# jfjell/Octree-Raymarcher

Hardware: AMD Instinct MI355X
Metric: Mrays/s (primary+shadow) at 1920x1080, depth-12 SVO (higher is better)
Workload: dtype f32; 1 GPU; c3_1080p_depth12_4x1x4_shadow; depth_per_chunk=12, chunksize=128, nodes=99473656, bricks=34206642, hbm_pool_bytes=11087035656, kernel=auto, launches_in_flight=2, frames_per_launch=16, frames_in_flight=32, gather=False, partition=single, ranks_seen=1, launcher=single process

## Files before the change

octree-raymarcher_amd/csrc/device.hip:

```cpp
#include <hip/hip_runtime.h>

#include <algorithm>
#include <cmath>
#include <cstdlib>
#include <chrono>
#include <cstring>
#include <mutex>
#include <new>
#include <string>
#include <vector>

#include "kernel_literal.hip.h"
#include "kernel_stack.hip.h"
#include "see_through.hip.h"
#include "local_shadows.hip.h"
#include "shadowmap.hip.h"
#include "locate.hip.h"
#include "ao.hip.h"
#include "hit_voxels.hip.h"
#include "hip_own.h"
#include "wide_tree.hip.h"

using namespace svo;

// ... 567 lines not shown
        uint64_t tl = std::min<uint64_t>(tree_left, desc->trees), tr = std::min<uint64_t>(std::max(tree_right, tree_left), desc->trees);
        uint64_t bl = std::min<uint64_t>(twig_left, desc->twigs), br = std::min<uint64_t>(std::max(twig_right, twig_left), desc->twigs);
        if (desc->trees > old_trees) { tl = std::min(tl, old_trees); tr = desc->trees; }
        if (desc->twigs > old_twigs) { bl = std::min(bl, old_twigs); br = desc->twigs; }
        const uint64_t keep_t = std::min(tr, old_trees), keep_b = std::min(br, old_twigs);
        std::vector<uint32_t> undo_t(cur.tree.begin() + (ptrdiff_t)std::min(tl, keep_t), cur.tree.begin() + (ptrdiff_t)keep_t);
        std::vector<uint16_t> undo_b(cur.twig.begin() + (ptrdiff_t)(std::min(bl, keep_b) * TWIG_WORDS), cur.twig.begin() + (ptrdiff_t)(keep_b * TWIG_WORDS));
        cur.tree.resize(desc->trees);
        cur.twig.resize(desc->twigs * TWIG_WORDS);
        if (tl < tr) std::memcpy(cur.tree.data() + tl, desc->tree + tl, (tr - tl) * sizeof(uint32_t));
        if (bl < br) std::memcpy(cur.twig.data() + bl * TWIG_WORDS, desc->twig + bl * TWIG_WORDS, (br - bl) * TWIG_WORDS * sizeof(uint16_t));
        const uint64_t cap_t0 = cur.tree_capacity, cap_b0 = cur.twig_capacity;
        cur.fit_capacity(cur.tree.size(), cur.twig_count());
        rc = validate_chunk(cur, why);
        if (rc != SVO_OK) {
            cur.tree.resize(old_trees); cur.twig.resize(old_twigs * TWIG_WORDS);
            std::copy(undo_t.begin(), undo_t.end(), cur.tree.begin() + (ptrdiff_t)std::min(tl, keep_t));
            std::copy(undo_b.begin(), undo_b.end(), cur.twig.begin() + (ptrdiff_t)(std::min(bl, keep_b) * TWIG_WORDS));
            cur.tree_capacity = cap_t0; cur.twig_capacity = cap_b0;
            set_error("svo_world_update: " + why); return rc;
        }
        tree_left = tl; tree_right = tr; twig_left = bl; twig_right = br;
    } else {
        ChunkPools next;
        std::memcpy(next.position, desc->position, sizeof next.position);
        next.size = desc->size; next.depth = desc->depth;
        next.tree.assign(desc->tree, desc->tree + desc->trees);
        if (desc->twigs) next.twig.assign(desc->twig, desc->twig + desc->twigs * TWIG_WORDS);
        next.tree_capacity = cur.tree_capacity;
        next.twig_capacity = cur.twig_capacity;
        next.fit_capacity(next.tree.size(), next.twig_count());
        rc = validate_chunk(next, why);
        if (rc != SVO_OK) { set_error("svo_world_update: " + why); return rc; }
        if (next.size != (float)w->chunksize) { set_error("svo_world_update: chunk size must equal chunksize"); return SVO_ERR_UNSUPPORTED; }
        cur.tree.swap(next.tree);
        cur.twig.swap(next.twig);
        cur.twigs_on_device = 0;
        cur.trees_on_device = 0;
        std::memcpy(cur.position, next.position, sizeof cur.position);
        cur.size = next.size; cur.depth = next.depth;
        cur.tree_capacity = next.tree_capacity; cur.twig_capacity = next.twig_capacity;
        if (realloc_ || desc->trees != old_trees || desc->twigs != old_twigs) { tree_left = 0; tree_right = desc->trees; twig_left = 0; twig_right = desc->twigs; }
    }
    classify_world(*w);
    if (w->device < 0) return SVO_OK;
    return install_chunk(*w, chunk, cur.tree.data(), cur.twig.data(), hipMemcpyHostToDevice, tree_left, tree_right, twig_left, twig_right);
}

}

extern "C" {

int svo_world_upload(svo_world *w, int device)
{
    try { return world_upload_impl(w, device); }
    catch (const std::bad_alloc &) { set_error("svo_world_upload: out of host memory"); return SVO_ERR_OUT_OF_MEMORY; }
    catch (...) { set_error("svo_world_upload: unexpected exception"); return SVO_ERR_HIP; }
}

int svo_world_update(svo_world *w, int chunk, const svo_chunk_desc *desc,
                     uint64_t tree_left, uint64_t tree_right, uint64_t twig_left, uint64_t twig_right, int realloc_)
{
    try { return world_update_impl(w, chunk, desc, tree_left, tree_right, twig_left, twig_right, realloc_); }
    catch (const std::bad_alloc &) { set_error("svo_world_update: out of host memory"); return SVO_ERR_OUT_OF_MEMORY; }
    catch (...) { set_error("svo_world_update: unexpected exception"); return SVO_ERR_HIP; }
}

}

namespace svo {

constexpr int STACK_REFILL = 8;
constexpr int STACK_WAVES = 6;
using StackKernel = void (*)(TraceArgs);
template <int MAXLV, bool BIG, bool GLSL, bool SEG> constexpr StackKernel stack_kernel = k_trace_stack<MAXLV, STACK_REFILL, STACK_WAVES, BIG, GLSL, SEG>;
constexpr int STACK_CLASSES = 12;
#define STACK_PAIR(MAXLV, BIG, SEG) stack_kernel<MAXLV, BIG, true, SEG>, stack_kernel<MAXLV, BIG, false, SEG>
#define STACK_SET(SEG) STACK_PAIR(10, true, SEG), STACK_PAIR(22, true, SEG), STACK_PAIR(6, false, SEG), STACK_PAIR(10, false, SEG), STACK_PAIR(16, false, SEG), STACK_PAIR(22, false, SEG)
static const StackKernel STACK_KERNELS[] = { STACK_SET(false), STACK_SET(true) };
#undef STACK_SET
#undef STACK_PAIR
static_assert(sizeof(STACK_KERNELS) / sizeof(StackKernel) == 2 * STACK_CLASSES, "an unbounded and a bounded instantiation per class");
static_assert(sizeof(STACK_KERNELS) / sizeof(StackKernel) == sizeof(Hbm::stack_blocks) / sizeof(int), "one grid size per instantiation");

}

extern "C" {

static float world_min(const svo_world *w, int a) { return (float)(w->chunkcoordmin[a] * (int)(float)w->chunksize); }
static V3 miss_ray_origin(const svo_world *w)
{
    const float cs = (float)w->chunksize;
    return V3{ world_min(w, 0), world_min(w, 1) - (float)w->height * cs - cs, world_min(w, 2) - (float)w->depth * cs - cs };
}

static int fill_common(svo_world *w, const svo_trace_params *prm, TraceArgs &A)
{
    if (!w) return SVO_ERR_INVALID_ARG;
    if (prm && prm->see_through > 0xFFFFu) { set_error("svo_trace: see_through is a 16-bit material"); return SVO_ERR_INVALID_ARG; }
    if (w->device < 0) { set_error("svo_trace: world is not uploaded"); return SVO_ERR_NOT_UPLOADED; }
    std::memset(&A, 0, sizeof A);
    const float cs = (float)w->chunksize;
    const int dims[3] = { w->width, w->height, w->depth };
    for (int a = 0; a < 3; ++a) {
        A.worldmin[a] = world_min(w, a);
        A.worldmax[a] = (float)(w->chunkcoordmin[a] + dims[a]) * cs;
    }
    A.chunksize = cs;
    A.inv_chunksize = 1.0f / cs;
    A.dimw = w->width; A.dimh = w->height; A.dimd = w->depth;
    for (int a = 0; a < 3; ++a) {
        A.ccm[a] = w->chunkcoordmin[a];
        A.cbase[a] = positive_mod(w->chunkcoordmin[a], dims[a]);
    }
    A.chunks = w->hbm->chunks.p; A.tree = w->hbm->tree.p; A.twig = w->hbm->twig.p; A.mask = w->hbm->mask.p;
    A.wchunks = w->hbm->wchunks.p; A.wide = w->hbm->wide.p; A.wbase = w->hbm->wbase.p; A.bmat = w->hbm->bmat.p;
    if (prm && prm->semantics != SVO_SEMANTICS_CPU && prm->semantics != SVO_SEMANTICS_GLSL) { set_error("svo_trace: unknown semantics"); return SVO_ERR_INVALID_ARG; }
    const bool glsl = prm && prm->semantics == SVO_SEMANTICS_GLSL;
    A.glsl = glsl ? 1 : 0;
    A.eps = (prm && prm->eps != 0.0f) ? prm->eps : (glsl ? 1.0f / 4096.0f : 1.0f / 8192.0f);
    A.cap_chunk = (prm && prm->max_chunk_steps > 0) ? prm->max_chunk_steps : (glsl ? 256 : 1000);
    A.cap_tree = (prm && prm->max_tree_steps > 0) ? prm->max_tree_steps : (glsl ? 512 : 1000);
    A.cap_twig = (prm && prm->max_twig_steps > 0) ? prm->max_twig_steps : (glsl ? 64 : 1000);
    A.guard_eps = glsl ? A.eps : -INFINITY;
    A.leaf_back = glsl ? 0.0f : A.eps;
    A.shadow = (prm && prm->shadow) ? 1 : 0;
    A.normal_mode = (prm && prm->normal_mode == SVO_NORMAL_FACE) ? SVO_NORMAL_FACE : SVO_NORMAL_CUBE;
    float l[3] = { 1.0f, -1.0f, 0.0f };
    if (prm && (prm->light_dir[0] != 0.0f || prm->light_dir[1] != 0.0f || prm->light_dir[2] != 0.0f))
        std::memcpy(l, prm->light_dir, sizeof l);
    const float nx = -l[0], ny = -l[1], nz = -l[2];
    const float inv = 1.0f / std::sqrt(nx * nx + ny * ny + nz * nz);
    A.sdir[0] = nx * inv; A.sdir[1] = ny * inv; A.sdir[2] = nz * inv;
    A.counters = prm ? prm->counters_dev : nullptr;
    A.exact_geometry = w->exact_geometry ? 1 : 0;
    A.tile_cost = prm ? prm->tile_cost_dev : nullptr;
    A.tile_order = prm ? prm->tile_order_dev : nullptr;
    A.work = w->hbm->work.p;
    return SVO_OK;
}

static bool stack_needs_big(const svo_world *w)
{
#ifdef SVO_FORCE_WIDE64
    return true;
#else
    return w->wide_pool_cap * 64 >= (1ull << 30) || w->twig_pool_cap >= (1ull << 29);
#endif
}

static int pick_kernel(const svo_world *w, const svo_trace_params *prm, const TraceArgs &A)
{
    const int want = prm ? prm->kernel : SVO_KERNEL_AUTO;
    const bool stack_ok = w->exact_geometry && w->max_levels <= (int)WIDE_MAX_LEVELS && w->wide_ok && w->twig_pool_cap < (1ull << 32);
    if (want == SVO_KERNEL_LITERAL) return SVO_KERNEL_LITERAL;
    if (want == SVO_KERNEL_STACK) {
        if (!stack_ok) { set_error("svo_trace: SVO_KERNEL_STACK needs exact geometry, chunk depth <= 24 and the world's wide trees (svo_world_info.wide_nodes)"); return SVO_ERR_UNSUPPORTED; }
        return SVO_KERNEL_STACK;
    }
    if (want != SVO_KERNEL_AUTO) { set_error("svo_trace: unknown kernel id"); return SVO_ERR_INVALID_ARG; }
    return (stack_ok && !A.counters) ? SVO_KERNEL_STACK : SVO_KERNEL_LITERAL;
}

static int launch_stack(svo_world *w, const TraceArgs &A, int tiles_per_wave, int in_flight, hipStream_t s)
{
    const int lv = w->max_levels;
    const int depth = stack_needs_big(w) ? (lv <= 10 ? 0 : 1) : lv <= 6 ? 2 : lv <= 10 ? 3 : lv <= 16 ? 4 : 5;
    const int which = 2 * depth + (A.glsl ? 0 : 1) + (A.tmax ? STACK_CLASSES : 0);
    const StackKernel kernel = STACK_KERNELS[which];
    int &resident = w->hbm->stack_blocks[which];
    if (resident <= 0) {
        hipDeviceProp_t prop;
        if (hipGetDeviceProperties(&prop, w->device) != hipSuccess) return SVO_ERR_HIP;
        int per_cu = 0;
        if (hipOccupancyMaxActiveBlocksPerMultiprocessor(&per_cu, kernel, 64, 0) != hipSuccess || per_cu <= 0) per_cu = 16;
        resident = prop.multiProcessorCount * per_cu;
#ifdef SVO_TEST_HOOKS
        if (const char *cap = std::getenv("SVO_GRID_WAVES_PER_CU")) { const int c = std::atoi(cap); if (c > 0) resident = prop.multiProcessorCount * std::min(c, per_cu); }
#endif
    }
    const int64_t per_wave = tiles_per_wave > 1 ? tiles_per_wave : 1;
    const int64_t tiles = (int64_t)A.ntiles * (A.nframes > 0 ? A.nframes : 1);
    const int64_t slots = in_flight >= 2 ? std::max<int64_t>(1, (int64_t)resident * 2 / in_flight) : resident;
    const int blocks = (int)std::min<int64_t>((tiles + per_wave - 1) / per_wave, slots);
    hipLaunchKernelGGL(kernel, dim3((unsigned)blocks), dim3(64), 0, s, A);
    return SVO_OK;
}

static int use_view(svo_world *w, uint32_t m, TraceArgs &A, hipStream_t s)
{
    Hbm &d = *w->hbm;
    if (d.view_material != m) {
        const uint64_t n4 = w->wide_pool_len * 16, bricks = w->twig_pool_len;
        if (!d.view_wide.p) {
            if (d.view_wide.alloc(std::max<uint64_t>(n4, 1) * 4, w->device) != hipSuccess ||
                d.view_mask.alloc(std::max<uint64_t>(bricks, 1), w->device) != hipSuccess) {
                d.view_wide = Pooled<uint32_t>();
                set_error("svo_trace: hipMalloc of the see-through view failed"); return SVO_ERR_OUT_OF_MEMORY;
            }
        } else {
            for (Event &e : d.work_done) if (e.e) if (const int rc = e.wait(s)) return rc;
        }
        d.view_material = 0;
        if ((n4 + 255) / 256 > 0x7FFFFFFFull || (bricks * 8 + 255) / 256 > 0x7FFFFFFFull) { set_error("svo_trace: pools too large for one view launch"); return SVO_ERR_UNSUPPORTED; }
        if (n4) hipLaunchKernelGGL(k_view_wide, dim3((unsigned)((n4 + 255) / 256)), dim3(256), 0, s, reinterpret_cast<const uint4 *>(d.wide.p),
                                   reinterpret_cast<uint4 *>(d.view_wide.p), n4, m);
        if (bricks) hipLaunchKernelGGL(k_view_mask, dim3((unsigned)((bricks * 8 + 255) / 256)), dim3(256), 0, s, d.twig.p, d.mask.p, d.view_mask.p, bricks, m);
        HIP_TRY(hipGetLastError());
        if (const int rc = d.view_built.record(s)) return rc;
        d.view_material = m;
    } else {
        if (const int rc = d.view_built.wait(s)) return rc;
    }
    A.wide = d.view_wide.p;
    A.mask = d.view_mask.p;
    return SVO_OK;
}

static int launch(svo_world *w, const svo_trace_params *prm, TraceArgs &A, hipStream_t s)
{
    const int kernel = pick_kernel(w, prm, A);
    if (kernel < 0) return kernel;
    HIP_TRY(hipSetDevice(w->device));
    const uint32_t see = prm ? prm->see_through : 0u;
    if (see && kernel == SVO_KERNEL_STACK) {
        const int rc = use_view(w, see, A, s);
        if (rc != SVO_OK) return rc;
    }
    Hbm &d = *w->hbm;
    d.work_last = d.work_next;
    d.work_next = (d.work_next + 1) % WORK_SLOTS;
    A.work = d.work.p + WORK_SLOT_WORDS * d.work_last;
    Event &ev = d.work_done[d.work_last];
    if (const int rc = ev.wait(s)) return rc;
    HIP_TRY(hipMemsetAsync(A.work, 0, WORK_SLOT_WORDS * sizeof(unsigned long long), s));
    if (A.n <= 0) return ev.record(s) == SVO_OK ? SVO_OK : SVO_ERR_HIP;
    if (kernel == SVO_KERNEL_LITERAL) {
        const int64_t blocks = (A.n + 255) / 256;
        if (blocks > 0x7FFFFFFF) { set_error("svo_trace: too many rays for one launch"); return SVO_ERR_UNSUPPORTED; }
        const auto literal = see ? (A.tmax ? k_trace_literal<true, true> : k_trace_literal<true, false>) : (A.tmax ? k_trace_literal<false, true> : k_trace_literal<false, false>);
        hipLaunchKernelGGL(literal, dim3((unsigned)blocks), dim3(256), 0, s, A, see);
    } else {
        if (A.ntiles > (1 << 25)) { set_error("svo_trace: more than 2^31 rays in one stack-kernel launch"); return SVO_ERR_UNSUPPORTED; }
        if (A.tile_cost) HIP_TRY(hipMemsetAsync(A.tile_cost, 0, (size_t)A.ntiles * (size_t)(A.from_camera ? A.nframes : 1) * 2 * sizeof(uint32_t), s));
        const int rc = launch_stack(w, A, prm ? prm->tiles_per_wave : 0, prm ? prm->launches_in_flight : 0, s);
        if (rc != SVO_OK) { set_error("svo_trace: device query failed"); return rc; }
    }
    HIP_TRY(hipGetLastError());
    return ev.record(s);
}

static int fill_cameras(const svo_camera *cams, int nframes, TraceArgs &A)
{
    if (!cams || nframes < 1 || nframes > MAX_FRAMES) { set_error("svo_trace: between 1 and 16 cameras per launch"); return SVO_ERR_INVALID_ARG; }
    for (int f = 0; f < nframes; ++f) {
        const svo_camera &c = cams[f];
        if (c.width <= 0 || c.height <= 0) { set_error("svo_trace: bad camera"); return SVO_ERR_INVALID_ARG; }
        if (c.width != cams[0].width || c.height != cams[0].height) { set_error("svo_trace_frames: the cameras of one launch share one image size"); return SVO_ERR_INVALID_ARG; }
        A.cams[f] = frame_cam(c);
    }
    A.from_camera = 1;
    A.nframes = nframes;
    A.imgw = cams[0].width; A.imgh = cams[0].height;
    return SVO_OK;
}

static int launch_frames(svo_world *w, const svo_trace_params *prm, TraceArgs &A, const char *who, hipStream_t s)
{
    A.n = (int64_t)A.w * A.h;
    A.tiles_per_row = (A.w + TILE_W - 1) / TILE_W;
    const int64_t tiles = (int64_t)A.tiles_per_row * ((A.h + TILE_H - 1) / TILE_H);
    if (tiles * A.nframes > 0x3FFFFFFF || A.n * A.nframes > 0x7FFFFFFF) { set_error(std::string(who) + ": image too large"); return SVO_ERR_UNSUPPORTED; }
    A.ntiles = (int32_t)tiles;
    if (A.nframes == 1) return launch(w, prm, A, s);
    const int kernel = pick_kernel(w, prm, A);
    if (kernel < 0) return kernel;
    if (kernel == SVO_KERNEL_STACK) return launch(w, prm, A, s);
    if (prm && prm->counters_dev) { set_error(std::string(who) + ": work counters are per launch of one frame"); return SVO_ERR_UNSUPPORTED; }
    const int nframes = A.nframes;
    char *out = static_cast<char *>(A.out);
    for (int f = 0; f < nframes; ++f) {
        TraceArgs F = A;
        F.nframes = 1; F.cams[0] = A.cams[f];
        F.out = out + (size_t)f * (size_t)A.n * sizeof(svo_hit);
        const int rc = launch(w, prm, F, s);
        if (rc != SVO_OK) return rc;
    }
    return SVO_OK;
}

int svo_trace_frames(svo_world *w, const svo_camera *cams, int nframes, const svo_trace_params *prm,
                     int x0, int y0, int rw, int rh, svo_hit *out_dev, void *stream)
{
    TraceArgs A;
    int rc = fill_common(w, prm, A);
    if (rc != SVO_OK) return rc;
    if ((rc = fill_cameras(cams, nframes, A)) != SVO_OK) return rc;
    if (!out_dev || rw < 0 || rh < 0 || x0 < 0 || y0 < 0) { set_error("svo_trace: bad rectangle or output"); return SVO_ERR_INVALID_ARG; }
    A.x0 = x0; A.y0 = y0; A.w = rw; A.h = rh;
    A.bh = rh > 0 ? rh : 1; A.ystep = 0;
    A.out = out_dev;
    return launch_frames(w, prm, A, "svo_trace", (hipStream_t)stream);
}

int svo_trace(svo_world *w, const svo_camera *cam, const svo_trace_params *prm,
              int x0, int y0, int rw, int rh, svo_hit *out_dev, void *stream)
{
    return svo_trace_frames(w, cam, 1, prm, x0, y0, rw, rh, out_dev, stream);
}

// ... 354 lines not shown
```

octree-raymarcher_amd/csrc/kernel_stack.hip.h:

```cpp
#pragma once
#include "march.hip.h"
#include "step_asm.hip.h"

namespace svo {

constexpr int CW_ESCAPE_PENDING = (int)0x80000000;
enum : int { M_DONE = 0, M_WORLD = 1, M_HIT = 2, M_TREE = 3, M_TWIG = 4 };

constexpr int VOTE_WORLD = 8;
constexpr int VOTE_HIT = 16;
constexpr int VOTE_BUSY = 24;
constexpr int CREEP_SERIOUS = 6;
constexpr int CREEP_LANES = 8;
#define SVO_LIKELY(x) __builtin_expect(!!(x), 1)
#define SVO_UNLIKELY(x) __builtin_expect(!!(x), 0)
constexpr int STEP_EXTRA = 4;
constexpr int STEP_LANES = 8;
constexpr int DRAIN_STEPS = 8;
#ifndef SVO_SURE_MISS_WHEN
#define SVO_SURE_MISS_WHEN __builtin_amdgcn_readfirstlane(more ? 0 : 1)
#endif

__device__ __forceinline__ float recip_pow2(float x) { return __uint_as_float(0x7F000000u - __float_as_uint(x)); }

__device__ __forceinline__ int chunk_index_pow2(const TraceArgs &A, V3 p)
{
    float qx = p.x * A.inv_chunksize, qy = p.y * A.inv_chunksize, qz = p.z * A.inv_chunksize;
    if (qx < 0.0f) qx -= 1.0f;
    if (qy < 0.0f) qy -= 1.0f;
    if (qz < 0.0f) qz -= 1.0f;
    const int ix = (int)qx, iy = (int)qy, iz = (int)qz;
    const int rx = ix - A.ccm[0], ry = iy - A.ccm[1], rz = iz - A.ccm[2];
    int mx = A.cbase[0] + rx, my = A.cbase[1] + ry, mz = A.cbase[2] + rz;
    mx -= (mx >= A.dimw) ? A.dimw : 0; mx += (mx < 0) ? A.dimw : 0;
    my -= (my >= A.dimh) ? A.dimh : 0; my += (my < 0) ? A.dimh : 0;
    mz -= (mz >= A.dimd) ? A.dimd : 0; mz += (mz < 0) ? A.dimd : 0;
    return my * A.dimw * A.dimd + mz * A.dimw + mx;
}

__device__ __forceinline__ V3 cube_normal_pow2(V3 s, V3 lo, float size, float eps)
{
    const V3 hi = lo + size;
    const V3 c = (lo + hi) * 0.5f;
    const V3 p = s - c;
    const float d = fabsf(lo.x - hi.x) * 0.5f;
    const float invd = recip_pow2(d);
    const float b = 1.0f + eps;
    const float ix = (float)(int)((p.x * invd) * b), iy = (float)(int)((p.y * invd) * b), iz = (float)(int)((p.z * invd) * b);
    const float dot = ix * ix + iy * iy + iz * iz;
    float inv;
    if (dot == 1.0f) inv = 1.0f;
    else if (dot == 2.0f) inv = __uint_as_float(0x3F3504F3u);
    else if (dot == 3.0f) inv = __uint_as_float(0x3F13CD3Au);
    else inv = 1.0f / sqrtf(dot);
    return mk(ix * inv, iy * inv, iz * inv);
}

__device__ __forceinline__ uint32_t child_slot(int ux, int uy, int uz, int sh)
{
    const uint32_t bx = __builtin_amdgcn_ubfe((uint32_t)ux, (uint32_t)sh, 1u);
    const uint32_t by = __builtin_amdgcn_ubfe((uint32_t)uy, (uint32_t)sh, 1u);
    const uint32_t bz = __builtin_amdgcn_ubfe((uint32_t)uz, (uint32_t)sh, 1u);
    return ((bz << 1) + by) * 2u + bx;
}
__device__ __forceinline__ uint32_t ld_node(const uint32_t *pool, uint32_t boff)
{
    return *reinterpret_cast<const uint32_t *>(reinterpret_cast<const char *>(pool) + (size_t)boff);
}
constexpr uint32_t WIDE_PAYLOAD = (1u << 25) - 1u;
__device__ __forceinline__ uint32_t wide_slot(int ux, int uy, int uz, int sh)
{
    const uint32_t bx = __builtin_amdgcn_ubfe((uint32_t)ux, (uint32_t)sh, 2u);
    const uint32_t by = __builtin_amdgcn_ubfe((uint32_t)uy, (uint32_t)sh, 2u);
    const uint32_t bz = __builtin_amdgcn_ubfe((uint32_t)uz, (uint32_t)sh, 2u);
    return (bz << 4) | (by << 2) | bx;
}
__device__ __forceinline__ bool is_branch(uint32_t word) { return (int32_t)word < (int32_t)0xC0000000; }

__device__ __forceinline__ TraceArgs args_reloaded()
{
    auto p = __builtin_amdgcn_kernarg_segment_ptr();
    asm volatile("" : "+s"(p));
    TraceArgs T;
    __builtin_memcpy(&T, p, sizeof T);
    return T;
}
__device__ __forceinline__ FrameCam camera_reloaded(int f)
{
    auto p = __builtin_amdgcn_kernarg_segment_ptr();
    asm volatile("" : "+s"(p));
    FrameCam c;
    __builtin_memcpy(&c, (decltype(p))((const char __attribute__((address_space(4))) *)p + __builtin_offsetof(TraceArgs, cams) + (size_t)f * sizeof(FrameCam)), sizeof c);
    return c;
}

__device__ __noinline__ float brick_layer_first_touch(int k, V3 a, V3 b, V3 g, V3 bmin, float r, unsigned long long mask)
{
    const float ak = k == 0 ? a.x : k == 1 ? a.y : a.z, bk = k == 0 ? b.x : k == 1 ? b.y : b.z, mk_ = k == 0 ? bmin.x : k == 1 ? bmin.y : bmin.z;
    const float au = k == 0 ? a.y : k == 1 ? a.z : a.x, av = k == 0 ? a.z : k == 1 ? a.x : a.y;
    const float gu = k == 0 ? g.y : k == 1 ? g.z : g.x, gv = k == 0 ? g.z : k == 1 ? g.x : g.y;
    const float mu = k == 0 ? bmin.y : k == 1 ? bmin.z : bmin.x, mv = k == 0 ? bmin.z : k == 1 ? bmin.x : bmin.y;
    const int su = k == 0 ? 4 : k == 1 ? 16 : 1, sv = k == 0 ? 16 : k == 1 ? 1 : 4;
    const float delta = r * 0.0625f;
    bool ok = (ak == mk_) & (bk < 0.0f);
    ok &= (mu >= 4.0f * r) & (mv >= 4.0f * r) & (delta >= (fabsf(mu) + fabsf(mv) + 8.0f * r) * 0x1p-21f);
    ok = ok && fabsf(gu) < 1.0e30f && fabsf(gv) < 1.0e30f;
    if (!ok) return -1.0f;
    const float u0 = au - mu, v0 = av - mv;
    float first = __uint_as_float(0x7F800000u);
    bool clean = true;
    for (int cv = 0; cv < 4; ++cv) {
        const float va = ((float)cv * r - delta - v0) * gv, vb = ((float)(cv + 1) * r + delta - v0) * gv;
        const float v_in = fminf(va, vb), v_out = fmaxf(va, vb);
        for (int cu = 0; cu < 4; ++cu) {
            const bool occupied = (mask >> (cu * su + cv * sv)) & 1ull;
            const float ua = ((float)cu * r - delta - u0) * gu, ub = ((float)(cu + 1) * r + delta - u0) * gu;
            const float s_in = fmaxf(fmaxf(fminf(ua, ub), v_in), 0.0f), s_out = fminf(fmaxf(ua, ub), v_out);
            clean &= (s_in == s_in) & (s_out == s_out);
            first = (occupied & (s_in <= s_out)) ? fminf(first, s_in) : first;
        }
    }
    return clean ? first * (1.0f - 0x1p-18f) : -1.0f;
}

__device__ __forceinline__ void note_tile_cost(int outk, uint32_t steps)
{
    const TraceArgs T = args_reloaded();
    if (!T.tile_cost) return;
    const int k = outk & 0x7FFFFFFF;
    int tile, frame = 0;
    if (T.from_camera) {
        const int per = T.w * T.h;
        frame = k / per;
        const int r = k - frame * per;
        const int ly = r / T.w, lx = r - ly * T.w;
        tile = (ly / TILE_H) * T.tiles_per_row + lx / TILE_W;
    } else tile = k >> 6;
    atomicMax(&T.tile_cost[((size_t)frame * (size_t)T.ntiles + (size_t)tile) * 2 + (outk < 0 ? 1 : 0)], steps);
}

template <bool GLSL>
__device__ __forceinline__ bool past_far_end(int mode, float t, float tt_saved, float tw, float eps, float far)
{
    const float tt = mode == M_TWIG ? tt_saved : t;
    return (mode == M_TREE || mode == M_TWIG) && tw + (GLSL ? tt : tt - eps) >= far;
}

template <int MAXLV, int REFILL, int WAVES_PER_SIMD, bool BIG, bool GLSL, bool SEG = false>
__global__ __launch_bounds__(64, WAVES_PER_SIMD) void k_trace_stack(TraceArgs A)
{
    __shared__ uint32_t stk[MAXLV / 2 + 1][64];
    __shared__ float tile_ray[SEG ? 12 : 11][64];
    constexpr int CHUNK_TAB = (BIG && MAXLV <= 10) ? 128 : 64;
    __shared__ uint32_t chunk_tab[6][CHUNK_TAB];
    stk[0][threadIdx.x] = 0u;
    const int lane = threadIdx.x;
    const bool want_cost = A.tile_cost != nullptr;
    const int n_chunks = A.dimw * A.dimh * A.dimd;
    const bool chunks_in_lds = n_chunks <= CHUNK_TAB;
    if (chunks_in_lds)
        for (int i = lane; i < n_chunks; i += 64) {
            const DevWide ch = A.wchunks[i];
            chunk_tab[0][i] = __float_as_uint(ch.bmin[0]); chunk_tab[1][i] = __float_as_uint(ch.bmin[1]); chunk_tab[2][i] = __float_as_uint(ch.bmin[2]);
            chunk_tab[3][i] = ch.levels; chunk_tab[4][i] = ch.wide_off; chunk_tab[5][i] = (uint32_t)ch.twig_off;
        }
    __syncthreads();
#ifdef SVO_STACK_TIMING
    const unsigned long long t_begin = __builtin_amdgcn_s_memrealtime();
    unsigned n_iters = 0, n_tree_lanes = 0, n_twig_lanes = 0, n_world_lanes = 0;
    unsigned n_world_runs = 0, n_hit_runs = 0, n_refill = 0, n_tilegen = 0, n_fix = 0;
    unsigned n_lane_twig = 0;
    unsigned n_lane_busy = 0;
    unsigned n_creep_runs = 0, n_creep_rounds = 0, n_dbg = 0;
    unsigned n_wsteps = 0, n_lsteps = 0, n_hit_wait = 0, n_dead_wait = 0, n_wsteps_b = 0, n_lsteps_b = 0, n_world_wait = 0, n_twig_b = 0;
#endif
    [[maybe_unused]] StepStats step_stats;

    const V3 wlo = ld3(A.worldmin), whi = ld3(A.worldmax);
    const V3 sdir = ld3(A.sdir);
    const V3 sg = recip(sdir);
    const float eps = A.eps;
    const bool eps_pow2 = (__float_as_uint(eps) & 0x807FFFFFu) == 0u && __float_as_uint(eps) >= 0x00800000u && __float_as_uint(eps) < 0x7F800000u;
    const float csize = A.chunksize;

    const int tr_cols = A.tiles_per_row;
    const int tr_rows = A.ntiles / (tr_cols > 0 ? tr_cols : 1);
    const bool by_cols = tr_cols >= TILE_REGIONS;
    const int reg_q = (by_cols ? tr_cols : tr_rows) / TILE_REGIONS, reg_rem = (by_cols ? tr_cols : tr_rows) % TILE_REGIONS;
    int region = (int)(__builtin_amdgcn_s_getreg(20 | (0 << 6) | (3 << 11)) & (TILE_REGIONS - 1));
    int regions_left = TILE_REGIONS;
    int tile_first = 0;
    int tile_next = 64;
    bool more = true;
    unsigned rays_marched = 0;

    int mode = M_DONE;
    int outk = 0;
    V3 alpha = mk(0, 0, 0), beta = mk(0, 0, 1), g = mk(0, 0, 0);
    float tw = 0.0f;
    [[maybe_unused]] float far = __uint_as_float(0x7F800000u);
    int cw = 0;
    uint32_t guard = 0;
    V3 O = mk(0, 0, 0), Blo = mk(0, 0, 0);
    float res = 1.0f, t = 0.0f;
    int cnt = 0;
    float tt_saved = 0.0f, t_miss = 0.0f;
    int it_saved = 0;
    V3 clo = mk(0, 0, 0);
    WideRef<BIG> wide_b = 0;
    auto ld_wide = [&](uint32_t e) -> uint32_t {
        if constexpr (BIG) return *reinterpret_cast<const uint32_t *>((size_t)wide_b + ((size_t)e << 2));
        else return ld_node(A.wide, wide_b + (e << 2));
    };
    uint32_t twig_off = 0;
    int levels = 0, ci = -1;
    int pux = 0, puy = 0, puz = 0, valid = 0, plev = 0;
    unsigned long long bmask = 0;
#ifndef SVO_CXX_STEP
    float bsize = 0.0f, res_tree = 1.0f;
    int nw_chunk = 1;
    const uint32_t lds_lane = (uint32_t)(size_t)(__attribute__((address_space(3))) uint32_t *)&stk[0][lane];
    StepUniform SU;
    SU.csize = csize; SU.eps = eps; SU.eps2 = 2.0f * eps; SU.cap_twig = A.cap_twig; SU.wide = A.wide; SU.mask = A.mask; SU.descend_shift = MAXLV <= 10 ? DESCEND_SHIFT_SHALLOW : DESCEND_SHIFT_DEEP;
#endif
    int creepn = 0;
    for (;;) {
        unsigned long long dead = __ballot(mode == M_DONE);
        while (more && __popcll(dead) >= REFILL) {
            if (tile_next >= 64) {
                int t32 = -1, tcol = 0, trow = 0, tframe = 0;
                const uint32_t *order = args_reloaded().tile_order;
                if (order) {
                    regions_left = 0;
                    unsigned long long tix = 0;
                    if (lane == 0) tix = atomicAdd(&A.work[WORK_CURSOR0], 1ull);
                    int t = __builtin_amdgcn_readfirstlane((int)tix);
                    if (t < A.ntiles * A.nframes) {
                        tframe = t / A.ntiles; t -= tframe * A.ntiles;
                        t32 = (int)order[t];
                        if ((uint32_t)t32 >= (uint32_t)A.ntiles) { t32 = 0; tframe = -1; }
                        trow = t32 / tr_cols; tcol = t32 - trow * tr_cols;
                    }
                }
                while (regions_left > 0) {
                    const int span = reg_q + (region < reg_rem ? 1 : 0);
                    const int first = region * reg_q + (region < reg_rem ? region : reg_rem);
                    const int count = span * (by_cols ? tr_rows : tr_cols);
                    unsigned long long tix = 0;
                    if (lane == 0) tix = atomicAdd(&A.work[WORK_CURSOR0 + region], 1ull);
                    int t = __builtin_amdgcn_readfirstlane((int)tix);
                    if (t < count * A.nframes) {
                        if (A.nframes > 1) { tframe = t / count; t -= tframe * count; }
                        if (by_cols) { trow = t / span; tcol = first + (t - trow * span); }
                        else { trow = first + t / tr_cols; tcol = t % tr_cols; }
                        t32 = trow * tr_cols + tcol;
                        break;
                    }
                    region = (region + 1) & (TILE_REGIONS - 1);
                    --regions_left;
                }
                if (t32 < 0) { more = false; break; }
                tile_first = t32 * 64;
                tile_next = 0;
#ifdef SVO_STACK_TIMING
                ++n_tilegen;
#endif
                {
                    const TraceArgs T = args_reloaded();
                    const int id = tile_first + lane;
                    bool ok;
                    int k = -1;
                    V3 o = mk(0, 0, 0), d = mk(0, 0, 1);
                    if (T.from_camera) {
                        const int lx = tcol * TILE_W + (lane & (TILE_W - 1));
                        const int ly = trow * TILE_H + lane / TILE_W;
                        ok = (lx < T.w) & (ly < T.h) & (tframe >= 0);
                        k = (tframe * T.h + ly) * T.w + lx;
                        int px = 0, py = 0;
                        if (ok) local_to_pixel(T, lx, ly, px, py);
                        if (ok && (py >= T.imgh || px >= T.imgw)) { store_miss(A.out, k, 0); ok = false; }
                        if (ok) camera_ray(camera_reloaded(tframe), T.imgw, T.imgh, px, py, o, d);
                    } else {
                        ok = id < T.n && tframe >= 0;
                        k = id;
                        if (ok) { o = ld3(T.origins + 3 * (long long)id); d = ld3(T.dirs + 3 * (long long)id); }
                        if constexpr (SEG) tile_ray[11][lane] = ok ? T.tmax[id] : 0.0f;
                    }
                    const V3 gg = recip(d);
                    float t0 = 0.0f;
                    if (ok) {
                        bool hit = true;
                        if (!inside(o, wlo, whi)) t0 = (GLSL ? enter_glsl(o, gg, wlo, whi, hit) : enter(o, d, wlo, whi, hit)) + eps;
                        rays_marched++;
                        if (!hit) { store_miss(A.out, k, 0); ok = false; }
                    }
                    tile_ray[0][lane] = o.x; tile_ray[1][lane] = o.y; tile_ray[2][lane] = o.z;
                    tile_ray[3][lane] = d.x; tile_ray[4][lane] = d.y; tile_ray[5][lane] = d.z;
                    tile_ray[6][lane] = gg.x; tile_ray[7][lane] = gg.y; tile_ray[8][lane] = gg.z;
                    tile_ray[9][lane] = t0;
                    tile_ray[10][lane] = __int_as_float(ok ? k : -1);
                    __syncthreads();
                }
            }
#ifdef SVO_STACK_TIMING
            ++n_refill;
#endif
            const int rank = (int)__builtin_amdgcn_mbcnt_hi((unsigned)(dead >> 32), __builtin_amdgcn_mbcnt_lo((unsigned)dead, 0u));
            const int avail = 64 - tile_next;
            if (mode == M_DONE && rank < avail) {
                const int slot = tile_next + rank;
                const int k = __float_as_int(tile_ray[10][slot]);
                if (k >= 0) {
                    outk = k;
                    alpha = mk(tile_ray[0][slot], tile_ray[1][slot], tile_ray[2][slot]);
                    beta = mk(tile_ray[3][slot], tile_ray[4][slot], tile_ray[5][slot]);
                    g = mk(tile_ray[6][slot], tile_ray[7][slot], tile_ray[8][slot]);
                    tw = tile_ray[9][slot];
                    if constexpr (SEG) far = tile_ray[11][slot];
                    cw = 0; guard = 0; creepn = 0;
                    mode = M_WORLD;
                }
            }
            const int ndead = __popcll(dead);
            tile_next += (ndead < avail) ? ndead : avail;
            __syncthreads();
            dead = __ballot(mode == M_DONE);
        }
        if (dead == ~0ull) break;
#ifdef SVO_STACK_TIMING
        ++n_iters;
        n_tree_lanes += __popcll(__ballot(mode == M_TREE)); n_twig_lanes += __popcll(__ballot(mode == M_TWIG));
        n_world_lanes += __popcll(__ballot(mode == M_WORLD));
#endif

        const int n_busy = __popcll(__ballot(mode == M_TREE || mode == M_TWIG));
        const int n_world = __popcll(__ballot(mode == M_WORLD));
        const int n_hit = __popcll(__ballot(mode == M_HIT));
        const bool run_world = n_world > 0 && (n_world >= VOTE_WORLD || n_busy < VOTE_BUSY ||
                                               __ballot(mode == M_WORLD && creepn <= -CREEP_SERIOUS) != 0ull);
        const bool run_hit = n_hit > 0 && (n_hit >= VOTE_HIT || n_busy < VOTE_BUSY);

        if (SVO_UNLIKELY(mode != M_DONE && mode != M_HIT && ++guard > STEP_GUARD)) {
            if (outk < 0) store_flags(A.out, outk & 0x7FFFFFFF, SVO_HIT_FLAG | SVO_SHADOW_TRACED | SVO_ERR_FLAG | (A.normal_mode == SVO_NORMAL_FACE ? (uint32_t)SVO_FACE_NORMAL : 0u));
            else store_miss(A.out, outk, SVO_ERR_FLAG);
            mode = M_DONE;
        }

#ifdef SVO_STACK_TIMING
        n_world_runs += run_world; n_hit_runs += run_hit;
#endif
        if (run_world && mode == M_WORLD) {
            if (cw < 0) {
                cw &= ~CW_ESCAPE_PENDING;
                if constexpr (GLSL) tw += guarded(escape(O, g, clo, clo + csize), eps) + eps;
                else tw += escape(O, g, clo, clo + csize) + eps;
            }
            bool miss = cw >= A.cap_chunk;
            if constexpr (SEG) miss |= (GLSL ? tw : tw - eps) >= far;
            if (!miss) {
                cw++;
                const V3 p = alpha + beta * tw;
                miss = !inside(p, wlo, whi);
                if (!miss) {
                    const int ci_new = chunk_index_pow2(A, p);
                    if (ci_new != ci) { valid = 0; pux = 0; puy = 0; puz = 0; }
                    ci = ci_new;
                    uint32_t ch_levels, ch_wide, ch_twig;
                    if (chunks_in_lds) {
                        clo = mk(__uint_as_float(chunk_tab[0][ci]), __uint_as_float(chunk_tab[1][ci]), __uint_as_float(chunk_tab[2][ci]));
                        ch_levels = chunk_tab[3][ci]; ch_wide = chunk_tab[4][ci]; ch_twig = chunk_tab[5][ci];
                    } else {
                        const DevWide ch = A.wchunks[ci];
                        clo = ld3(ch.bmin);
                        ch_levels = ch.levels; ch_wide = ch.wide_off; ch_twig = (uint32_t)ch.twig_off;
                    }
                    bool contained = inside(p, clo, clo + csize);
                    if (GLSL && !contained) tw += guarded(escape(p, g, clo, clo + csize), eps) + eps;
                    else miss = !contained;
                    if (contained) {
                        if constexpr (BIG) wide_b = (unsigned long long)(size_t)A.wide + ((unsigned long long)ch_wide << 8);
                        else wide_b = ch_wide << 8;
                        twig_off = ch_twig;
                        levels = (int)ch_levels;
                        O = p; t = 0.0f; cnt = A.cap_tree;
                        Blo = clo;
                        res = csize * __uint_as_float((uint32_t)(127 - levels) << 23);
#ifndef SVO_CXX_STEP
                        bsize = csize; res_tree = res; nw_chunk = levels ? (levels + 1) >> 1 : 1;
#endif
                        mode = M_TREE;
                    }
                }
            }
            if (miss) {
                if (outk >= 0) store_miss(A.out, outk, 0);
                if (want_cost) note_tile_cost(outk, guard);
                mode = M_DONE;
            }
        }

        int pass = 0;
        const int fixed_steps = (n_busy >= STEP_LANES && __ballot(creepn > 0 || creepn <= -4 * CREEP_SERIOUS) == 0ull) ? STEP_EXTRA : 0;
        for (;;) {
#ifdef SVO_STACK_TIMING
        n_lane_twig += mode == M_TWIG ? (pass == 0 ? 1u + (unsigned)fixed_steps : (unsigned)DRAIN_STEPS) : 0u;
        n_lane_busy += (mode == M_TREE || mode == M_TWIG) ? (pass == 0 ? 1u + (unsigned)fixed_steps : (unsigned)DRAIN_STEPS) : 0u;
        { const int nm = __popcll(__ballot(mode == M_TREE || mode == M_TWIG)); n_wsteps += nm > 0; n_lsteps += nm; if (more) { n_wsteps_b += nm > 0; n_lsteps_b += nm; n_hit_wait += __popcll(__ballot(mode == M_HIT)); n_dead_wait += __popcll(__ballot(mode == M_DONE)); n_world_wait += __popcll(__ballot(mode == M_WORLD)); n_twig_b += __popcll(__ballot(mode == M_TWIG)); } }
#endif
#ifndef SVO_CXX_STEP
        const int nsteps = pass == 0 ? 1 + fixed_steps : DRAIN_STEPS;
        const int sure_miss = SVO_SURE_MISS_WHEN;
        march_steps_asm<BIG, GLSL>(mode, O, Blo, bsize, res, t, cnt, tt_saved, t_miss, it_saved, tw, cw, pux, puy, puz, valid, plev, bmask, creepn,
                                   beta, g, clo, alpha, levels, nw_chunk, res_tree, wide_b, twig_off, lds_lane, SU, nsteps | (sure_miss << 16), step_stats);
        pass += nsteps - 1;
#else
        if (mode == M_TREE || mode == M_TWIG) {
            enum : int { S_LEAVE = 0, S_ADVANCE = 1, S_ENTER = 2, S_HIT_LEAF = 3, S_HIT_CELL = 4, S_BAD = 5 };
            const bool twig = mode == M_TWIG;
            const float Bsize = twig ? res * 4.0f : csize, inv_res = recip_pow2(res);
            const int crept = creepn < 0 ? -creepn : creepn;
            creepn = -crept;
            bool leave = cnt <= 0;
            cnt -= 1;
            const V3 p = O + beta * t;
            leave |= !inside(p, Blo, Blo + Bsize);
            const float fx = (p.x - Blo.x) * inv_res, fy = (p.y - Blo.y) * inv_res, fz = (p.z - Blo.z) * inv_res;
            int ux = (int)fx, uy = (int)fy, uz = (int)fz;
#ifdef SVO_STACK_TIMING
            n_fix += __ballot(!twig && ((fx == (float)ux) | (fy == (float)uy) | (fz == (float)uz))) != 0;
#endif
            if (SVO_UNLIKELY(!twig && ((fx == (float)ux) | (fy == (float)uy) | (fz == (float)uz)))) {
                const int nmax = (1 << levels) - 1;
                ux = ux > nmax ? nmax : ux; uy = uy > nmax ? nmax : uy; uz = uz > nmax ? nmax : uz;
                ux -= (Blo.x + (float)ux * res > p.x) ? 1 : 0;
                uy -= (Blo.y + (float)uy * res > p.y) ? 1 : 0;
                uz -= (Blo.z + (float)uz * res > p.z) ? 1 : 0;
            }
            if (twig) leave |= (ux > 3) | (uy > 3) | (uz > 3);

            int what = S_LEAVE;
            int low = 0;
            uint32_t payload = 0;
            if (SVO_LIKELY(!leave)) {
                if (!twig) {
                    const uint32_t diff = (uint32_t)((ux ^ pux) | (uy ^ puy) | (uz ^ puz));
                    const int nw = levels ? (levels + 1) >> 1 : 1;
                    const int hb = 32 - __clz((int)(diff | 1u));
                    const int keep = nw - ((hb + 1) >> 1);
                    int k;
                    asm("v_med3_i32 %0, %1, 0, %2" : "=v"(k) : "v"(keep), "v"(valid));
                    uint32_t wnode = stk[k][lane];
                    int sh = 2 * (nw - 1 - k);
                    uint32_t word = ld_wide((wnode << 6) + wide_slot(ux, uy, uz, sh));
                    while (is_branch(word)) {
                        wnode = word & WIDE_PAYLOAD;
                        ++k;
                        stk[k][lane] = wnode;
                        sh -= 2;
                        word = ld_wide((wnode << 6) + wide_slot(ux, uy, uz, sh));
                    }
                    valid = k; pux = ux; puy = uy; puz = uz;
                    plev = (int)((word >> 25) & 31u);
                    low = (1 << (levels - plev)) - 1;
                    const uint32_t type = node_type(word);
                    what = type == EMPTY ? S_ADVANCE : type == LEAF ? S_HIT_LEAF : S_ENTER;
                    payload = word;
                } else {
                    payload = (uint32_t)(uz * 16 + uy * 4 + ux);
                    what = ((bmask >> payload) & 1ull) ? S_HIT_CELL : S_ADVANCE;
                }
            }

            if (what == S_ADVANCE || what == S_ENTER) {
                const V3 E_lo = mk(Blo.x + (float)(ux & ~low) * res, Blo.y + (float)(uy & ~low) * res, Blo.z + (float)(uz & ~low) * res);
                const float E_size = res * (float)(low + 1);
                const float e = (GLSL ? guarded(escape(p, g, E_lo, E_lo + E_size), eps) : escape(p, g, E_lo, E_lo + E_size)) + eps;
                if (what == S_ADVANCE) {
                    t += e;
                    creepn = e < 2.0f * eps ? crept + 1 : 0;
                } else {
                    bmask = A.mask[twig_off + (payload & WIDE_PAYLOAD)];
                    tt_saved = t; t_miss = t + e; it_saved = cnt;
                    O = p; t = 0.0f; cnt = A.cap_twig;
                    Blo = E_lo;
                    res = E_size * 0.25f;
                    mode = M_TWIG;
                }
            }
            if (leave) {
                if (twig) {
                    t = t_miss;
                    cnt = it_saved;
                    O = alpha + beta * tw;
                    Blo = clo;
                    res = csize * __uint_as_float((uint32_t)(127 - levels) << 23);
                    mode = M_TREE;
                } else {
                    cw |= CW_ESCAPE_PENDING;
                    mode = M_WORLD;
                }
            }
            if (what == S_HIT_LEAF) {
                tw = tw + (GLSL ? t : t - eps);
                cnt = (int)SVO_CELL_NONE;
                mode = M_HIT;
            }
            if (what == S_HIT_CELL) {
                float sdist = t;
                sdist += tt_saved;
                tw = tw + sdist;
                cnt = (int)payload;
                mode = M_HIT;
            }
        }
#endif

        ++pass;
        if (pass <= fixed_steps) continue;
        if (more || pass >= 256) break;
        const unsigned long long marching = __ballot(mode == M_TREE || mode == M_TWIG);
        if (marching == 0ull || marching != __ballot(mode != M_DONE) || __ballot(creepn > 0 || creepn <= -4 * CREEP_SERIOUS) != 0ull) break;
        if constexpr (SEG) if (__ballot(past_far_end<GLSL>(mode, t, tt_saved, tw, eps, far)) != 0ull) break;
        }
        guard += pass - 1;
        if constexpr (SEG) {
            if (past_far_end<GLSL>(mode, t, tt_saved, tw, eps, far)) {
                if (mode == M_TWIG) O = alpha + beta * tw;
                creepn = creepn > 0 ? -creepn : creepn;
                cw |= CW_ESCAPE_PENDING;
                mode = M_WORLD;
            }
        }

#include "creep_block.inc"

        if (mode == M_HIT && outk < 0) {
            store_flags(A.out, outk & 0x7FFFFFFF, SVO_HIT_FLAG | SVO_SHADOW_TRACED | SVO_SHADOWED | (A.normal_mode == SVO_NORMAL_FACE ? (uint32_t)SVO_FACE_NORMAL : 0u));
            if (want_cost) note_tile_cost(outk, guard);
            mode = M_DONE;
        }
        if constexpr (SEG) {
            if (mode == M_HIT && !(tw < far)) {
                store_miss(A.out, outk, 0);
                if (want_cost) note_tile_cost(outk, guard);
                mode = M_DONE;
            }
        }
        if (run_hit && mode == M_HIT) {
            const int nw = levels ? (levels + 1) >> 1 : 1;
            const uint32_t wn = valid > 0 ? stk[valid][lane] : 0u, slot = wide_slot(pux, puy, puz, 2 * (nw - 1 - valid));
            const uint32_t word = ld_wide((wn << 6) + slot);
            uint32_t node = 0u;
            if (plev != 0) {
                const uint32_t ci = ((slot >> 1) & 1u) | ((slot >> 2) & 2u) | ((slot >> 3) & 4u);
                const uint32_t gi = (slot & 1u) | ((slot >> 1) & 2u) | ((slot >> 2) & 4u);
                size_t wnode_in_pool;
                if constexpr (BIG) wnode_in_pool = (((size_t)wide_b - (size_t)A.wide) >> 8) + wn;
                else wnode_in_pool = (wide_b >> 8) + wn;
                const uint32_t *wb = A.wbase + wnode_in_pool * WIDE_BASE_WORDS;
                const int level_child = 2 * valid + 1 - (2 * nw - levels);
                node = plev == level_child ? wb[0] + ci : wb[1 + ci] + gi;
            }
            const uint32_t hitc = (uint32_t)cnt;
            V3 vlo;
            float vsize;
            uint32_t material;
            if (hitc == SVO_CELL_NONE) {
                const int low = (1 << (levels - plev)) - 1;
                vlo = mk(Blo.x + (float)(pux & ~low) * res, Blo.y + (float)(puy & ~low) * res, Blo.z + (float)(puz & ~low) * res);
                vsize = res * (float)(low + 1);
                material = word & 0xFFFFu;
            } else {
                vlo = mk(Blo.x + (float)(hitc & 3u) * res, Blo.y + (float)((hitc >> 2) & 3u) * res, Blo.z + (float)(hitc >> 4) * res);
                vsize = res;
                const unsigned long long brick = (unsigned long long)twig_off + (word & WIDE_PAYLOAD);
                material = A.bmat[brick];
                if (material == 0xFFFFu) material = A.twig[brick * TWIG_WORDS + hitc];
            }
            const V3 point = alpha + beta * (tw - eps);
            const bool face = A.normal_mode == SVO_NORMAL_FACE;
            const V3 n = face ? face_normal(point, vlo, vlo + vsize, beta) : cube_normal_pow2(point, vlo, vsize, eps);
            const uint32_t flags = SVO_HIT_FLAG | (A.shadow ? SVO_SHADOW_TRACED : 0u) | (face ? (uint32_t)SVO_FACE_NORMAL : 0u);
            store_hit(A.out, outk, tw, n, material, flags, (uint32_t)ci, node, hitc);
            if (want_cost) note_tile_cost(outk, guard);
            mode = M_DONE;
            if (A.shadow) {
                alpha = point; beta = sdir; g = sg;
                outk |= (int)0x80000000;
                if constexpr (SEG) far = __uint_as_float(0x7F800000u);
                tw = 0.0f; cw = 0; guard = 0; creepn = 0;
                bool hit = true;
                if (!inside(alpha, wlo, whi)) tw = (GLSL ? enter_glsl(alpha, g, wlo, whi, hit) : enter(alpha, beta, wlo, whi, hit)) + eps;
                mode = hit ? M_WORLD : M_DONE;
                rays_marched++;
            }
        }
    }

    unsigned total = rays_marched;
    for (int off = 32; off > 0; off >>= 1) total += __shfl_down(total, off, 64);
    if (lane == 0 && total) atomicAdd(&A.work[1], (unsigned long long)total);
#ifdef SVO_STACK_TIMING
    unsigned busiest = n_lane_busy;
    for (int off = 32; off > 0; off >>= 1) busiest = max(busiest, (unsigned)__shfl_xor((int)busiest, off, 64));
    unsigned busiest_twig = n_lane_busy == busiest ? n_lane_twig : 0u;
    for (int off = 32; off > 0; off >>= 1) busiest_twig = max(busiest_twig, (unsigned)__shfl_xor((int)busiest_twig, off, 64));
    if (lane == 0 && A.counters) {
        uint4 c; c.x = (uint32_t)t_begin; c.y = (uint32_t)__builtin_amdgcn_s_memrealtime(); c.z = n_iters; c.w = total;
        reinterpret_cast<uint4 *>(A.counters)[6 * blockIdx.x] = c;
        uint4 e; e.x = n_world_runs | (n_hit_runs << 16); e.y = n_refill | (n_tilegen << 12) | (n_fix << 20); e.z = n_tree_lanes; e.w = n_twig_lanes | (n_world_lanes << 20);
        reinterpret_cast<uint4 *>(A.counters)[6 * blockIdx.x + 1] = e;
        uint4 f; f.x = n_creep_runs | (busiest_twig << 16); f.y = busiest; f.z = n_creep_rounds; f.w = n_dbg;
        reinterpret_cast<uint4 *>(A.counters)[6 * blockIdx.x + 2] = f;
        uint4 h; h.x = n_wsteps; h.y = n_lsteps; h.z = n_hit_wait; h.w = n_dead_wait;
        reinterpret_cast<uint4 *>(A.counters)[6 * blockIdx.x + 3] = h;
        uint4 h2; h2.x = n_wsteps_b; h2.y = n_lsteps_b; h2.z = n_world_wait; h2.w = n_twig_b;
        reinterpret_cast<uint4 *>(A.counters)[6 * blockIdx.x + 4] = h2;
        uint4 h3; h3.x = step_stats.steps; h3.y = step_stats.lanes; h3.z = step_stats.stalls; h3.w = step_stats.chased;
        reinterpret_cast<uint4 *>(A.counters)[6 * blockIdx.x + 5] = h3;
    }
#endif
}

}
```

Baseline: 7371 Mrays/s.

## Streamline stack kernel scheduling votes and chunk lookup with uniform branches and u24 math

Moves the chunk-grid parameters into a 32-byte LDS struct and computes the chunk index with a branchless single wrap and v_mad_u32_u24. A host-side limit of fewer than 2^24 chunks keeps the 24-bit multiply valid. Ballot popcounts are pinned to scalar registers and the world and hit phases are restructured into wave-uniform outer branches, which is meant to cut VALU and SGPR-to-VGPR overhead in the scheduler loop. The chunk table size shrinks slightly for some variants to make room for the struct, and the hit path's node lookup is turned into a single indexed load.

```diff
diff --git a/octree-raymarcher_amd/csrc/device.hip b/octree-raymarcher_amd/csrc/device.hip
--- a/octree-raymarcher_amd/csrc/device.hip
+++ b/octree-raymarcher_amd/csrc/device.hip
@@ -743,10 +743,11 @@
 static int pick_kernel(const svo_world *w, const svo_trace_params *prm, const TraceArgs &A)
 {
     const int want = prm ? prm->kernel : SVO_KERNEL_AUTO;
-    const bool stack_ok = w->exact_geometry && w->max_levels <= (int)WIDE_MAX_LEVELS && w->wide_ok && w->twig_pool_cap < (1ull << 32);
+    const bool stack_ok = w->exact_geometry && w->max_levels <= (int)WIDE_MAX_LEVELS && w->wide_ok && w->twig_pool_cap < (1ull << 32) &&
+                          (long long)w->width * w->height * w->depth < (1ll << 24);
     if (want == SVO_KERNEL_LITERAL) return SVO_KERNEL_LITERAL;
     if (want == SVO_KERNEL_STACK) {
-        if (!stack_ok) { set_error("svo_trace: SVO_KERNEL_STACK needs exact geometry, chunk depth <= 24 and the world's wide trees (svo_world_info.wide_nodes)"); return SVO_ERR_UNSUPPORTED; }
+        if (!stack_ok) { set_error("svo_trace: SVO_KERNEL_STACK needs exact geometry, chunk depth <= 24, fewer than 2^24 chunks and the world's wide trees (svo_world_info.wide_nodes)"); return SVO_ERR_UNSUPPORTED; }
         return SVO_KERNEL_STACK;
     }
     if (want != SVO_KERNEL_AUTO) { set_error("svo_trace: unknown kernel id"); return SVO_ERR_INVALID_ARG; }
diff --git a/octree-raymarcher_amd/csrc/kernel_stack.hip.h b/octree-raymarcher_amd/csrc/kernel_stack.hip.h
--- a/octree-raymarcher_amd/csrc/kernel_stack.hip.h
+++ b/octree-raymarcher_amd/csrc/kernel_stack.hip.h
@@ -23,19 +23,46 @@
 
 __device__ __forceinline__ float recip_pow2(float x) { return __uint_as_float(0x7F000000u - __float_as_uint(x)); }
 
-__device__ __forceinline__ int chunk_index_pow2(const TraceArgs &A, V3 p)
-{
-    float qx = p.x * A.inv_chunksize, qy = p.y * A.inv_chunksize, qz = p.z * A.inv_chunksize;
+__device__ __forceinline__ unsigned long long vote(bool p) { return __builtin_amdgcn_ballot_w64(p); }
+__device__ __forceinline__ int vote_count(unsigned long long m)
+{
+    int n = (int)__popcll(m);
+    asm("" : "+s"(n));
+    return n;
+}
+
+struct ChunkGrid {
+    float inv;
+    int32_t off[3];
+    int32_t dimw, dimh, dimd;
+    uint32_t table_in_lds;
+};
+static_assert(sizeof(ChunkGrid) == 32, "two 16-byte LDS reads");
+
+__device__ __forceinline__ int wrap_once(int m, int dim)
+{
+    const uint32_t a = (uint32_t)m, b = (uint32_t)(m + dim), c = (uint32_t)(m - dim);
+    return (int)min(min(a, b), c);
+}
+
+__device__ __forceinline__ void chunk_cell_pow2(const ChunkGrid &G, V3 p, int &mx, int &my, int &mz)
+{
+    float qx = p.x * G.inv, qy = p.y * G.inv, qz = p.z * G.inv;
     if (qx < 0.0f) qx -= 1.0f;
     if (qy < 0.0f) qy -= 1.0f;
     if (qz < 0.0f) qz -= 1.0f;
     const int ix = (int)qx, iy = (int)qy, iz = (int)qz;
-    const int rx = ix - A.ccm[0], ry = iy - A.ccm[1], rz = iz - A.ccm[2];
-    int mx = A.cbase[0] + rx, my = A.cbase[1] + ry, mz = A.cbase[2] + rz;
-    mx -= (mx >= A.dimw) ? A.dimw : 0; mx += (mx < 0) ? A.dimw : 0;
-    my -= (my >= A.dimh) ? A.dimh : 0; my += (my < 0) ? A.dimh : 0;
-    mz -= (mz >= A.dimd) ? A.dimd : 0; mz += (mz < 0) ? A.dimd : 0;
-    return my * A.dimw * A.dimd + mz * A.dimw + mx;
+    mx = wrap_once(ix + G.off[0], G.dimw); my = wrap_once(iy + G.off[1], G.dimh); mz = wrap_once(iz + G.off[2], G.dimd);
+}
+__device__ __forceinline__ uint32_t mad_u24(uint32_t a, uint32_t b, uint32_t c)
+{
+    uint32_t r;
+    asm("v_mad_u32_u24 %0, %1, %2, %3" : "=v"(r) : "v"(a), "v"(b), "v"(c));
+    return r;
+}
+__device__ __forceinline__ int chunk_index_u24(const ChunkGrid &G, int mx, int my, int mz)
+{
+    return (int)mad_u24(mad_u24((uint32_t)my, (uint32_t)G.dimd, (uint32_t)mz), (uint32_t)G.dimw, (uint32_t)mx);
 }
 
 __device__ __forceinline__ V3 cube_normal_pow2(V3 s, V3 lo, float size, float eps)
@@ -151,13 +178,20 @@
 {
     __shared__ uint32_t stk[MAXLV / 2 + 1][64];
     __shared__ float tile_ray[SEG ? 12 : 11][64];
-    constexpr int CHUNK_TAB = (BIG && MAXLV <= 10) ? 128 : 64;
+    constexpr int CHUNK_TAB = (BIG && MAXLV <= 10) ? 126 : MAXLV > 16 ? 62 : 64;
     __shared__ uint32_t chunk_tab[6][CHUNK_TAB];
+    __shared__ __attribute__((aligned(16))) ChunkGrid chunk_grid;
     stk[0][threadIdx.x] = 0u;
     const int lane = threadIdx.x;
     const bool want_cost = A.tile_cost != nullptr;
     const int n_chunks = A.dimw * A.dimh * A.dimd;
     const bool chunks_in_lds = n_chunks <= CHUNK_TAB;
+    if (lane == 0) {
+        chunk_grid.inv = A.inv_chunksize;
+        for (int a = 0; a < 3; ++a) chunk_grid.off[a] = A.cbase[a] - A.ccm[a];
+        chunk_grid.dimw = A.dimw; chunk_grid.dimh = A.dimh; chunk_grid.dimd = A.dimd;
+        chunk_grid.table_in_lds = chunks_in_lds ? 1u : 0u;
+    }
     if (chunks_in_lds)
         for (int i = lane; i < n_chunks; i += 64) {
             const DevWide ch = A.wchunks[i];
@@ -225,8 +259,8 @@
 #endif
     int creepn = 0;
     for (;;) {
-        unsigned long long dead = __ballot(mode == M_DONE);
-        while (more && __popcll(dead) >= REFILL) {
+        unsigned long long dead = vote(mode == M_DONE);
+        while (more && vote_count(dead) >= REFILL) {
             if (tile_next >= 64) {
                 int t32 = -1, tcol = 0, trow = 0, tframe = 0;
                 const uint32_t *order = args_reloaded().tile_order;
@@ -321,10 +355,10 @@
                     mode = M_WORLD;
                 }
             }
-            const int ndead = __popcll(dead);
+            const int ndead = vote_count(dead);
             tile_next += (ndead < avail) ? ndead : avail;
             __syncthreads();
-            dead = __ballot(mode == M_DONE);
+            dead = vote(mode == M_DONE);
         }
         if (dead == ~0ull) break;
 #ifdef SVO_STACK_TIMING
@@ -333,12 +367,13 @@
         n_world_lanes += __popcll(__ballot(mode == M_WORLD));
 #endif
 
-        const int n_busy = __popcll(__ballot(mode == M_TREE || mode == M_TWIG));
-        const int n_world = __popcll(__ballot(mode == M_WORLD));
-        const int n_hit = __popcll(__ballot(mode == M_HIT));
-        const bool run_world = n_world > 0 && (n_world >= VOTE_WORLD || n_busy < VOTE_BUSY ||
-                                               __ballot(mode == M_WORLD && creepn <= -CREEP_SERIOUS) != 0ull);
-        const bool run_hit = n_hit > 0 && (n_hit >= VOTE_HIT || n_busy < VOTE_BUSY);
+        const int n_busy = vote_count(vote(mode == M_TREE || mode == M_TWIG));
+        const int n_world = vote_count(vote(mode == M_WORLD));
+        const int n_hit = vote_count(vote(mode == M_HIT));
+        const bool few_busy = n_busy < VOTE_BUSY;
+        bool run_world = n_world >= (few_busy ? 1 : VOTE_WORLD);
+        if (!run_world && n_world > 0) run_world = vote(mode == M_WORLD && creepn <= -CREEP_SERIOUS) != 0ull;
+        const bool run_hit = n_hit >= (few_busy ? 1 : VOTE_HIT);
 
         if (SVO_UNLIKELY(mode != M_DONE && mode != M_HIT && ++guard > STEP_GUARD)) {
             if (outk < 0) store_flags(A.out, outk & 0x7FFFFFFF, SVO_HIT_FLAG | SVO_SHADOW_TRACED | SVO_ERR_FLAG | (A.normal_mode == SVO_NORMAL_FACE ? (uint32_t)SVO_FACE_NORMAL : 0u));
@@ -349,7 +384,8 @@
 #ifdef SVO_STACK_TIMING
         n_world_runs += run_world; n_hit_runs += run_hit;
 #endif
-        if (run_world && mode == M_WORLD) {
+        if (SVO_LIKELY(run_world)) { asm volatile("");
+        if (mode == M_WORLD) {
             if (cw < 0) {
                 cw &= ~CW_ESCAPE_PENDING;
                 if constexpr (GLSL) tw += guarded(escape(O, g, clo, clo + csize), eps) + eps;
@@ -362,11 +398,15 @@
                 const V3 p = alpha + beta * tw;
                 miss = !inside(p, wlo, whi);
                 if (!miss) {
-                    const int ci_new = chunk_index_pow2(A, p);
+                    const ChunkGrid G = chunk_grid;
+                    const bool table_in_lds = __builtin_amdgcn_readfirstlane((int)G.table_in_lds) != 0;
+                    int mx, my, mz;
+                    chunk_cell_pow2(G, p, mx, my, mz);
+                    const int ci_new = chunk_index_u24(G, mx, my, mz);
                     if (ci_new != ci) { valid = 0; pux = 0; puy = 0; puz = 0; }
                     ci = ci_new;
                     uint32_t ch_levels, ch_wide, ch_twig;
-                    if (chunks_in_lds) {
+                    if (table_in_lds) {
                         clo = mk(__uint_as_float(chunk_tab[0][ci]), __uint_as_float(chunk_tab[1][ci]), __uint_as_float(chunk_tab[2][ci]));
                         ch_levels = chunk_tab[3][ci]; ch_wide = chunk_tab[4][ci]; ch_twig = chunk_tab[5][ci];
                     } else {
@@ -397,10 +437,10 @@
                 if (want_cost) note_tile_cost(outk, guard);
                 mode = M_DONE;
             }
-        }
+        } }
 
         int pass = 0;
-        const int fixed_steps = (n_busy >= STEP_LANES && __ballot(creepn > 0 || creepn <= -4 * CREEP_SERIOUS) == 0ull) ? STEP_EXTRA : 0;
+        const int fixed_steps = (n_busy >= STEP_LANES && vote(creepn > 0 || creepn <= -4 * CREEP_SERIOUS) == 0ull) ? STEP_EXTRA : 0;
         for (;;) {
 #ifdef SVO_STACK_TIMING
         n_lane_twig += mode == M_TWIG ? (pass == 0 ? 1u + (unsigned)fixed_steps : (unsigned)DRAIN_STEPS) : 0u;
@@ -518,9 +558,9 @@
         ++pass;
         if (pass <= fixed_steps) continue;
         if (more || pass >= 256) break;
-        const unsigned long long marching = __ballot(mode == M_TREE || mode == M_TWIG);
-        if (marching == 0ull || marching != __ballot(mode != M_DONE) || __ballot(creepn > 0 || creepn <= -4 * CREEP_SERIOUS) != 0ull) break;
-        if constexpr (SEG) if (__ballot(past_far_end<GLSL>(mode, t, tt_saved, tw, eps, far)) != 0ull) break;
+        const unsigned long long marching = vote(mode == M_TREE || mode == M_TWIG);
+        if (marching == 0ull || marching != vote(mode != M_DONE) || vote(creepn > 0 || creepn <= -4 * CREEP_SERIOUS) != 0ull) break;
+        if constexpr (SEG) if (vote(past_far_end<GLSL>(mode, t, tt_saved, tw, eps, far)) != 0ull) break;
         }
         guard += pass - 1;
         if constexpr (SEG) {
@@ -546,7 +586,8 @@
                 mode = M_DONE;
             }
         }
-        if (run_hit && mode == M_HIT) {
+        if (run_hit) { asm volatile("");
+        if (mode == M_HIT) {
             const int nw = levels ? (levels + 1) >> 1 : 1;
             const uint32_t wn = valid > 0 ? stk[valid][lane] : 0u, slot = wide_slot(pux, puy, puz, 2 * (nw - 1 - valid));
             const uint32_t word = ld_wide((wn << 6) + slot);
@@ -559,7 +600,8 @@
                 else wnode_in_pool = (wide_b >> 8) + wn;
                 const uint32_t *wb = A.wbase + wnode_in_pool * WIDE_BASE_WORDS;
                 const int level_child = 2 * valid + 1 - (2 * nw - levels);
-                node = plev == level_child ? wb[0] + ci : wb[1 + ci] + gi;
+                const bool child = plev == level_child;
+                node = wb[child ? 0u : 1u + ci] + (child ? ci : gi);
             }
             const uint32_t hitc = (uint32_t)cnt;
             V3 vlo;
@@ -594,7 +636,7 @@
                 mode = hit ? M_WORLD : M_DONE;
                 rays_marched++;
             }
-        }
+        } }
     }
 
     unsigned total = rays_marched;
```

Result: faster. 7563 Mrays/s, median of 6 (+2.6%).
